# leabouffaut/DAS4Whales

Measured on AMD Instinct MI355X. Metric: channel-samples/sec through f-k filter + matched-filter, higher is better.
Workload: dtype f32 (matched filter: 2 x f16 split operands on the matrix cores, f32 accumulate); 1 GPU; 20000 channels x 120000 samples float32 per GPU, classic f-k fan mask (fk_filter_design defaults), stages fk+mf, HF+LF fin-call templates; api=public, parallelism=independent channel blocks x1

## Files before the change

das4whales_amd/csrc/mm_common.h:

```cpp
#pragma once
#include "fft_radix.h"

namespace d4w {

constexpr float kMmLoScale = 2048.f, kMmLoInv = 1.0f / 2048.f;

#ifdef D4W_EMU
typedef uint16_t mm_half;
struct alignas(16) mm_h8 { uint16_t v[8]; };
struct mm_f4 { float v[4]; };
__device__ __forceinline__ mm_half mm_to_half(float x) { return hipemu::f32_to_f16(x); }
__device__ __forceinline__ float mm_to_float(mm_half h) { return hipemu::f16_to_f32(h); }
__device__ __forceinline__ mm_f4 mm_zero() { return mm_f4{{0.f, 0.f, 0.f, 0.f}}; }
__device__ __forceinline__ mm_f4 mm_mfma(const mm_h8& a, const mm_h8& b, mm_f4 c) {
    hipemu::mfma_f32_16x16x32_f16(a.v, b.v, c.v);
    return c;
}
__device__ __forceinline__ float mm_get(const mm_f4& c, int r) { return c.v[r]; }
__device__ __forceinline__ void mm_set(mm_h8& a, int j, mm_half h) { a.v[j] = h; }
__device__ __forceinline__ int mm_uniform(int v) { return v; }
__device__ __forceinline__ void mm_sched_fence() {}
__device__ __forceinline__ void mm_store4(float* p, float a, float b, float c, float d) { p[0] = a; p[1] = b; p[2] = c; p[3] = d; }
__device__ __forceinline__ void mm_store1(float* p, float v) { *p = v; }
__device__ __forceinline__ float4 mm_load4_stream(const float4* p) { return *p; }
__device__ __forceinline__ void mm_put4(mm_half* p, const mm_half (&h)[4]) { p[0] = h[0]; p[1] = h[1]; p[2] = h[2]; p[3] = h[3]; }
__device__ __forceinline__ float mm_sqrt(float v) { return sqrtf(v); }
__device__ __forceinline__ void mm_wave_sync() { (void)__shfl_xor(0, 1); }
__device__ __forceinline__ float mm_clamp_half(float v) { return fminf(fmaxf(v, -65504.f), 65504.f); }
static inline int mm_num_cus() { return 2; }
#else
typedef _Float16 mm_half;
typedef _Float16 mm_h8 __attribute__((ext_vector_type(8)));
typedef _Float16 mm_h4 __attribute__((ext_vector_type(4)));
typedef float mm_f4 __attribute__((ext_vector_type(4)));
__device__ __forceinline__ mm_half mm_to_half(float x) { return (_Float16)x; }
__device__ __forceinline__ float mm_to_float(mm_half h) { return (float)h; }
__device__ __forceinline__ mm_f4 mm_zero() { mm_f4 z = {0.f, 0.f, 0.f, 0.f}; return z; }
__device__ __forceinline__ mm_f4 mm_mfma(mm_h8 a, mm_h8 b, mm_f4 c) { return __builtin_amdgcn_mfma_f32_16x16x32_f16(a, b, c, 0, 0, 0); }
__device__ __forceinline__ float mm_get(const mm_f4& c, int r) { return c[r]; }
__device__ __forceinline__ void mm_set(mm_h8& a, int j, mm_half h) { a[j] = h; }
__device__ __forceinline__ int mm_uniform(int v) { return __builtin_amdgcn_readfirstlane(v); }
__device__ __forceinline__ void mm_sched_fence() { __builtin_amdgcn_sched_barrier(0); }
__device__ __forceinline__ void mm_store4(float* p, float a, float b, float c, float d) {
    mm_f4 t = {a, b, c, d};
    __builtin_nontemporal_store(t, reinterpret_cast<mm_f4*>(p));
}
__device__ __forceinline__ void mm_store1(float* p, float v) { __builtin_nontemporal_store(v, p); }
__device__ __forceinline__ float4 mm_load4_stream(const float4* p) {
    const mm_f4 v = __builtin_nontemporal_load(reinterpret_cast<const mm_f4*>(p));
    return make_float4(v.x, v.y, v.z, v.w);
}
__device__ __forceinline__ void mm_put4(mm_half* p, const mm_half (&h)[4]) {
    mm_h4 v = {h[0], h[1], h[2], h[3]};
    *reinterpret_cast<mm_h4*>(p) = v;
}
__device__ __forceinline__ float mm_sqrt(float v) { return __builtin_amdgcn_sqrtf(v); }
__device__ __forceinline__ void mm_wave_sync() {
    __builtin_amdgcn_fence(__ATOMIC_RELEASE, "wavefront");
    __builtin_amdgcn_wave_barrier();
    __builtin_amdgcn_fence(__ATOMIC_ACQUIRE, "wavefront");
}
__device__ __forceinline__ float mm_clamp_half(float v) { return __builtin_amdgcn_fmed3f(v, -65504.f, 65504.f); }
static inline int mm_num_cus() {
    static int cached[64] = {0};
    int devid = 0, v = 0;
    if (hipGetDevice(&devid) != hipSuccess) return 256;
    if (devid >= 0 && devid < 64 && cached[devid] > 0) return cached[devid];
    if (hipDeviceGetAttribute(&v, hipDeviceAttributeMultiprocessorCount, devid) == hipSuccess && v > 0) {
        if (devid >= 0 && devid < 64) cached[devid] = v;
        return v;
    }
    return 256;
}
#endif

// ... 55 lines not shown
```

das4whales_amd/csrc/xcorr_mm.hip:

```cpp
#include <cstdlib>

#include "mm_common.h"

namespace d4w {

#ifndef D4W_MM_CH
#define D4W_MM_CH 4096
#endif
constexpr int kMmCH = D4W_MM_CH;
constexpr int kMmKS = 6;
constexpr int kMmKSLong = 8;
constexpr int kMmKSMax = 16;
constexpr int kMmSection = 32 * kMmKSMax - 16;
constexpr int kMmMaxSupport = 32 * kMmKSLong - 15;
constexpr int kMmMaxSections = 16;
constexpr int kMmThreads = 256;
template <int KSM>
struct MmGeom {
    static constexpr int Halo = 32 * KSM;
    static constexpr int Stage = kMmCH + Halo;
    static constexpr int Q = (Stage + 4 * kMmThreads - 1) / (4 * kMmThreads);
    static constexpr int LastQ = (Stage - (Q - 1) * 4 * kMmThreads) / 4;
    static constexpr int Arr = Stage + 8;
};
// ... 8 lines not shown
    float* y0;
    float* y1;
    int nx, ns, ld_next, n_next, ltaps, len0, len1;
    float* rowmax0;
    float* rowmax1;
    int clamp;
    int shift;
    int accumulate;
    float tail0, tail1;
};

__device__ __forceinline__ float mm_wave_scan(float v) {
#ifdef D4W_EMU
    const int lane = (int)(threadIdx.x & 63);
    for (int off = 1; off < 64; off <<= 1) {
        const float n = __shfl_up(v, (unsigned)off);
        if (lane >= off) v += n;
    }
    return v;
#else
    auto dpp = [](float x, auto ctrl, auto rmask) {
        return __int_as_float(__builtin_amdgcn_update_dpp(0, __float_as_int(x), decltype(ctrl)::value, decltype(rmask)::value, 0xf, false));
    };
    v += dpp(v, std::integral_constant<int, 0x111>{}, std::integral_constant<int, 0xf>{});
    v += dpp(v, std::integral_constant<int, 0x112>{}, std::integral_constant<int, 0xf>{});
    v += dpp(v, std::integral_constant<int, 0x114>{}, std::integral_constant<int, 0xf>{});
    v += dpp(v, std::integral_constant<int, 0x118>{}, std::integral_constant<int, 0xf>{});
    v += dpp(v, std::integral_constant<int, 0x142>{}, std::integral_constant<int, 0xa>{});
    v += dpp(v, std::integral_constant<int, 0x143>{}, std::integral_constant<int, 0xc>{});
    return v;
#endif
}

template <int KS0, int KS1, int WPS, bool TAIL = false, bool WMAX = false, bool WSPLIT = false>
__global__ __launch_bounds__(kMmThreads, WPS) void xcorr_mm_rows(MmArgs P) {
    static_assert(!(WSPLIT && KS1 > 0), "the wave-split kernel is the one-template code run by two wave pairs");
    constexpr int KSM = KS0 > KS1 ? KS0 : KS1;
    using GEO = MmGeom<KSM>;
    constexpr int kMmHalo = GEO::Halo, kMmStage = GEO::Stage, kMmQ = GEO::Q, kMmLastQ = GEO::LastQ, kMmArr = GEO::Arr;
    constexpr int kSeg = 4 * kMmQ;
    D4W_DYN_LDS(smem_raw);
    mm_half* lds = reinterpret_cast<mm_half*>(smem_raw);
    float* red = reinterpret_cast<float*>(lds + 4 * kMmArr);
    constexpr int kBlk = kMmCH / 4;
    float* pb = red + 8;
    float* wt = pb + 2 * kBlk;
    const int tid = (int)threadIdx.x;
    const int lane = tid & 63, wv = mm_uniform(tid >> 6);
    const int n16 = lane & 15, g = lane >> 4;
    const int ns = P.ns;
    const int tsel = WSPLIT ? (wv >> 1) : 0;

    const int nchunk = (ns + kMmCH - 1) / kMmCH;
    const long long total = (long long)P.nx * nchunk;
    const int nparts = min(8, (int)gridDim.x);
    const int xcd = (int)blockIdx.x % nparts, wq = (int)blockIdx.x / nparts, nq = ((int)gridDim.x - xcd + nparts - 1) / nparts;
    const long long lo_c = total * xcd / nparts, hi_c = total * (xcd + 1) / nparts;
    mm_h8 a0h[KS0], a0l[KS0];
    mm_h8 a1h[KS1 ? KS1 : 1], a1l[KS1 ? KS1 : 1];
    float osc0 = 1.f, osc1 = 1.f;
#ifdef D4W_MM_V_TAIL_DEALT
    constexpr bool kRows = false;
#else
    constexpr bool kRows = TAIL;
#endif
    auto next_chunk = [&](long long c) -> long long {
        if constexpr (kRows) {
            const long long r = c / nchunk;
            return (c - r * nchunk + 1 < nchunk) ? c + 1 : (r + (long long)gridDim.x) * nchunk;
        } else {
            return c + nq;
        }
    };
    const long long end_c = kRows ? total : hi_c;
    long long c_n = kRows ? (long long)blockIdx.x * nchunk : lo_c + wq;
    {
        float* tl = reinterpret_cast<float*>(smem_raw);
        constexpr int TLP = 16 + kMmHalo;
        for (int i = tid; i < 2 * TLP; i += kMmThreads) {
            const int t = i / TLP, u = i - t * TLP - 15;
            const int L = t ? P.len1 : P.len0;
            float tv = (u >= 0 && u < L && (t == 0 || KS1 > 0 || WSPLIT)) ? P.taps[(size_t)t * P.ltaps + u] : 0.f;
            if constexpr (TAIL) {
                if (u < L && (t == 0 || KS1 > 0 || WSPLIT)) tv += t ? P.tail1 : P.tail0;
            }
            tl[i] = tv;
        }
        __syncthreads();
        auto build = [&](const float* tp, int L, auto& ah, auto& al, auto ks, float& osc) {
            constexpr int KS = decltype(ks)::value;
            float m = 0.f;
            for (int i = lane; i < TLP; i += 64) m = fmaxf(m, fabsf(tp[i]));
            for (int o = 32; o > 0; o >>= 1) m = fmaxf(m, __shfl_xor(m, o));
            float up, down;
            mm_pow2_scale(m, up, down);
            osc = up;
            (void)L;
            static_for<KS>([&](auto kq) {
                constexpr int kk = decltype(kq)::value;
                static_for<8>([&](auto jq) {
                    constexpr int j = decltype(jq)::value;
                    const float v = tp[15 + 32 * kk + 8 * g + j - n16] * down;
                    mm_half hi, lo;
                    mm_split(v, hi, lo);
                    mm_set(ah[kk], j, hi);
                    mm_set(al[kk], j, lo);
                });
            });
        };
        build(tl + (WSPLIT ? tsel * TLP : 0), WSPLIT && tsel ? P.len1 : P.len0, a0h, a0l, std::integral_constant<int, KS0>{}, osc0);
        if constexpr (KS1 > 0) build(tl + TLP, P.len1, a1h, a1l, std::integral_constant<int, KS1>{}, osc1);
        __syncthreads();
    }

    float4 pre[kMmQ];
    Mean2 mu_n{0.f, 0.f};
    float g_n = 1.f;
    bool heavy_n = false;
    bool tail_n = false;
    int row_n = 0, c0_n = 0;

    auto issue = [&](long long c) {
        row_n = (int)(c / nchunk);
        c0_n = (int)(c - (long long)row_n * nchunk) * kMmCH;
        mu_n = mean2_load(P.mean, row_n);
        g_n = 1.f;
        const int s0 = c0_n + P.shift;
        tail_n = s0 + kMmStage > ns;
        if (P.maxabs) {
            const float a = P.maxabs[row_n];
            g_n = (a > 0.f) ? 1.0f / a : 0.f;
            heavy_n = fabsf(mu_n.hi) > 0.9921875f * a;
        }
        const float* xr = P.x + (size_t)row_n * ns;
        const bool al = (reinterpret_cast<uintptr_t>(xr + s0) & 15) == 0;
        if (al && s0 + kMmStage <= ns) {
            const float4* p = reinterpret_cast<const float4*>(xr + s0) + tid;
            static_for<kMmQ>([&](auto qq) {
                constexpr int q = decltype(qq)::value;
                if (q < kMmQ - 1 || tid < kMmLastQ) pre[q] = mm_load4_stream(p + q * kMmThreads);
            });
        } else {
            if (al && (ns & 3) == 0) {
                static_for<kMmQ>([&](auto qq) {
                    constexpr int q = decltype(qq)::value;
                    if (q < kMmQ - 1 || tid < kMmLastQ) {
                        const int i = s0 + 4 * (tid + q * kMmThreads);
                        const float4 v = *reinterpret_cast<const float4*>(xr + min(i, ns - 4));
                        pre[q] = (i < ns) ? v : make_float4(mu_n.hi, mu_n.hi, mu_n.hi, mu_n.hi);
                    }
                });
            } else {
                static_for<kMmQ>([&](auto qq) {
                    constexpr int q = decltype(qq)::value;
                    if (q < kMmQ - 1 || tid < kMmLastQ) {
                        const int i = s0 + 4 * (tid + q * kMmThreads);
                        const float a0 = xr[min(i, ns - 1)], a1 = xr[min(i + 1, ns - 1)], a2 = xr[min(i + 2, ns - 1)], a3 = xr[min(i + 3, ns - 1)];
                        pre[q] = make_float4(i < ns ? a0 : mu_n.hi, i + 1 < ns ? a1 : mu_n.hi, i + 2 < ns ? a2 : mu_n.hi, i + 3 < ns ? a3 : mu_n.hi);
                    }
                });
            }
            if (P.xnext && P.n_next > 0 && s0 + kMmStage > ns) {
                const float* xn = P.xnext + (size_t)row_n * P.ld_next;
                const int n_next = P.n_next;
                static_for<kMmQ>([&](auto qq) {
                    constexpr int q = decltype(qq)::value;
                    if (q < kMmQ - 1 || tid < kMmLastQ) {
                        const int d = s0 + 4 * (tid + q * kMmThreads) - ns;
                        const float b0 = xn[min(max(d, 0), n_next - 1)], b1 = xn[min(max(d + 1, 0), n_next - 1)];
                        const float b2 = xn[min(max(d + 2, 0), n_next - 1)], b3 = xn[min(max(d + 3, 0), n_next - 1)];
                        if (d >= 0 && d < n_next) pre[q].x = b0;
                        if (d + 1 >= 0 && d + 1 < n_next) pre[q].y = b1;
                        if (d + 2 >= 0 && d + 2 < n_next) pre[q].z = b2;
                        if (d + 3 >= 0 && d + 3 < n_next) pre[q].w = b3;
                    }
                });
            }
        }
    };

    if (c_n < end_c) issue(c_n);
    int buf = 0;
    constexpr bool want_max = WMAX;
    float pst_hi = 0.f, pst_lo = 0.f;
    for (long long c = c_n; c < end_c;) {
        const int row = row_n, c0 = c0_n;
        const Mean2 mu = mu_n;
        const bool tail = tail_n;
        const int n_valid = ns + ((P.xnext && P.n_next > 0) ? P.n_next : 0) - c0 - P.shift;
        float gsc = g_n, osx = 1.f;
        const float gout = g_n;
        const bool own_scale = !P.maxabs || heavy_n;
        mm_half* bh = lds + (size_t)buf * 2 * kMmArr;
        mm_half* bl = bh + kMmArr;
        const long long c_next = next_chunk(c);
        const int cin = c0 / kMmCH;
        if (TAIL && cin == 0) { pst_hi = 0.f; pst_lo = 0.f; }
        const float pst = pst_hi;
        if (own_scale) {
            float m = 0.f;
            static_for<kMmQ>([&](auto qq) {
                constexpr int q = decltype(qq)::value;
                if (q < kMmQ - 1 || tid < kMmLastQ) {
                    const float4 v = pre[q];
                    const int at = 4 * (tid + q * kMmThreads);
                    float d0 = demean(v.x, mu), d1 = demean(v.y, mu), d2 = demean(v.z, mu), d3 = demean(v.w, mu);
                    if (tail) {
                        if (at >= n_valid) d0 = 0.f;
                        if (at + 1 >= n_valid) d1 = 0.f;
                        if (at + 2 >= n_valid) d2 = 0.f;
                        if (at + 3 >= n_valid) d3 = 0.f;
                    }
                    m = fmaxf(fmaxf(m, fmaxf(fabsf(d0), fabsf(d1))), fmaxf(fabsf(d2), fabsf(d3)));
                }
            });
            for (int o = 32; o > 0; o >>= 1) m = fmaxf(m, __shfl_xor(m, o));
            if (lane == 0) red[wv + 4 * buf] = m;
            lds_barrier();
            m = fmaxf(fmaxf(red[4 * buf], red[4 * buf + 1]), fmaxf(red[4 * buf + 2], red[4 * buf + 3]));
            mm_pow2_scale(m, osx, gsc);
        }
        const float mlg = -mu.lo * gsc;
        static_for<kMmQ>([&](auto qq) {
            constexpr int q = decltype(qq)::value;
            float s[4] = {0.f, 0.f, 0.f, 0.f};
            const bool mine = q < kMmQ - 1 || tid < kMmLastQ;
            const int at = mm_pidx(4 * (tid + q * kMmThreads));
            if (mine) {
                const float4 v = pre[q];
#ifdef D4W_MM_V_FLOATMEAN
                s[0] = (v.x - mu.hi) * gsc; s[1] = (v.y - mu.hi) * gsc; s[2] = (v.z - mu.hi) * gsc; s[3] = (v.w - mu.hi) * gsc;
#else
                s[0] = fmaf(v.x - mu.hi, gsc, mlg); s[1] = fmaf(v.y - mu.hi, gsc, mlg); s[2] = fmaf(v.z - mu.hi, gsc, mlg); s[3] = fmaf(v.w - mu.hi, gsc, mlg);
#endif
                if (P.clamp && !own_scale) static_for<4>([&](auto ee) { constexpr int e = decltype(ee)::value; s[e] = mm_clamp_half(s[e]); });
                if (tail) {
                    const int a0 = 4 * (tid + q * kMmThreads);
                    static_for<4>([&](auto ee) { constexpr int e = decltype(ee)::value; if (a0 + e >= n_valid) s[e] = 0.f; });
                }
#ifdef D4W_MM_V_OLDSPLIT
                mm_half h[4], l[4];
                static_for<4>([&](auto ee) { constexpr int e = decltype(ee)::value; mm_split(s[e], h[e], l[e]); });
                mm_put4(bh + at, h);
                mm_put4(bl + at, l);
#else
                mm_split_put4(s, bh + at, bl + at);
#endif
            }
#ifdef D4W_MM_V_TAIL_NOSCAN
            if constexpr (false) {
#else
            if constexpr (TAIL && q < kMmCH / (4 * kMmThreads)) {
#endif
                const float t4 = (s[0] + s[1]) + (s[2] + s[3]);
                const float inc = mm_wave_scan(t4);
                pb[buf * kBlk + kMmThreads * q + tid] = inc - t4;
                if (lane == 63) wt[buf * 16 + 4 * q + wv] = inc;
            }
        });
        if (c_next < end_c) issue(c_next);
        lds_barrier();
        float* ya = ((WSPLIT && tsel) ? P.y1 : P.y0) + (size_t)row * ns;
        float* yb = KS1 ? P.y1 + (size_t)row * ns : nullptr;
        const bool valign = ((reinterpret_cast<uintptr_t>(ya + c0) & 15) == 0) && (!KS1 || (reinterpret_cast<uintptr_t>(yb + c0) & 15) == 0);
        const float oxs = (own_scale && P.maxabs) ? osx * gout : osx;
        const float o0 = osc0 * oxs, o1 = osc1 * oxs;
        float segoff = 0.f;
        constexpr int NTW = kMmCH / 256 / (WSPLIT ? 2 : 4), NST = NTW * KSM, PF = 2;
        auto tile_of = [&](int ti) { return WSPLIT ? (wv & 1) + 2 * ti : wv + 4 * ti; };
        auto frag = [&](const mm_half* arr, int T, int kk) -> mm_h8 {
            const int gr = 32 * T + 2 * n16 + g + 4 * kk;
            return *reinterpret_cast<const mm_h8*>(arr + mm_pidx(8 * gr));
        };
        mm_h8 fh[PF + 1], fl[PF + 1];
        static_for<PF>([&](auto ss) {
            constexpr int s_ = decltype(ss)::value;
            fh[s_] = frag(bh, tile_of(s_ / KSM), s_ % KSM);
            fl[s_] = frag(bl, tile_of(s_ / KSM), s_ % KSM);
        });
        mm_f4 c0h = mm_zero(), c0l = mm_zero(), c1h = mm_zero(), c1l = mm_zero();
        float vmax0 = -INFINITY, vmax1 = -INFINITY;
        float vsum = 0.f;
        static_for<NST>([&](auto ss) {
            constexpr int s_ = decltype(ss)::value, ti = s_ / KSM, kk = s_ % KSM;
            if constexpr (s_ + PF < NST) {
                fh[(s_ + PF) % (PF + 1)] = frag(bh, tile_of((s_ + PF) / KSM), (s_ + PF) % KSM);
                fl[(s_ + PF) % (PF + 1)] = frag(bl, tile_of((s_ + PF) / KSM), (s_ + PF) % KSM);
            }
            mm_sched_fence();
            const mm_h8 xh = fh[s_ % (PF + 1)], xl = fl[s_ % (PF + 1)];
            if constexpr (kk < KS0) {
                c0h = mm_mfma(a0h[kk], xh, c0h);
                c0l = mm_mfma(a0h[kk], xl, c0l);
            }
            if constexpr (kk < KS1) {
                c1h = mm_mfma(a1h[kk], xh, c1h);
                c1l = mm_mfma(a1h[kk], xl, c1l);
            }
            if constexpr (kk < KS0) c0l = mm_mfma(a0l[kk], xh, c0l);
            if constexpr (kk < KS1) c1l = mm_mfma(a1l[kk], xh, c1l);
            mm_sched_fence();
            if constexpr (kk == KSM - 1) {
                const int T = tile_of(ti);
                const int kl = 256 * T + 16 * n16 + 4 * g;
                const int k = c0 + kl;
                if constexpr (ti == 0) {
                if constexpr (TAIL) {
                    const float w = lane < 16 ? wt[buf * 16 + lane] : 0.f;
                    const float inc = mm_wave_scan(w);
                    segoff = inc - w;
        #ifdef D4W_EMU
                    const float own = __shfl(inc, 15);
        #else
                    const float own = __builtin_bit_cast(float, __builtin_amdgcn_readlane(__builtin_bit_cast(int, inc), 15));
        #endif
                    const double pd = ((double)pst_hi + (double)pst_lo) + (double)(own * oxs);
                    const float ph = (float)pd, pl2 = (float)(pd - (double)ph);
        #ifdef D4W_EMU
                    pst_hi = ph; pst_lo = pl2;
        #else
                    pst_hi = __builtin_bit_cast(float, __builtin_amdgcn_readfirstlane(__builtin_bit_cast(int, ph)));
                    pst_lo = __builtin_bit_cast(float, __builtin_amdgcn_readfirstlane(__builtin_bit_cast(int, pl2)));
        #endif
                }
                }
                float r0[4], r1[4];
                float a0 = 0.f, a1 = 0.f;
#ifdef D4W_MM_V_TAIL_NOSCAN
                if constexpr (false) {
#else
                if constexpr (TAIL) {
#endif
#ifdef D4W_EMU
                    const float so = __shfl(segoff, T);
#else
                    const float so = __builtin_bit_cast(float, __builtin_amdgcn_readlane(__builtin_bit_cast(int, segoff), T));
#endif
                    const float pbk = fmaf(so + pb[buf * kBlk + kMmThreads * (T >> 2) + 64 * (T & 3) + 4 * n16], oxs, pst);
                    a0 = ((WSPLIT && tsel) ? P.tail1 : P.tail0) * pbk;
                    a1 = P.tail1 * pbk;
                }
                static_for<4>([&](auto rr) {
                    constexpr int r = decltype(rr)::value;
                    r0[r] = fmaf(fmaf(mm_get(c0l, r), kMmLoInv, mm_get(c0h, r)), o0, a0);
                    if constexpr (KS1 > 0) r1[r] = fmaf(fmaf(mm_get(c1l, r), kMmLoInv, mm_get(c1h, r)), o1, a1);
                });
                c0h = mm_zero(); c0l = mm_zero(); c1h = mm_zero(); c1l = mm_zero();
                if (valign && k + 3 < ns) {
                    if (KS1 == 0 && P.accumulate) {
                        const float4 o = mm_load4_stream(reinterpret_cast<const float4*>(ya + k));
                        r0[0] += o.x; r0[1] += o.y; r0[2] += o.z; r0[3] += o.w;
                    }
                    mm_store4(ya + k, r0[0], r0[1], r0[2], r0[3]);
                    if constexpr (KS1 > 0) mm_store4(yb + k, r1[0], r1[1], r1[2], r1[3]);
                    if (want_max) {
                        vmax0 = fmaxf(vmax0, fmaxf(fmaxf(r0[0], r0[1]), fmaxf(r0[2], r0[3])));
#ifndef D4W_MM_V_NONAN
                        vsum += (r0[0] + r0[1]) + (r0[2] + r0[3]);
#endif
                        if constexpr (KS1 > 0) {
                            vmax1 = fmaxf(vmax1, fmaxf(fmaxf(r1[0], r1[1]), fmaxf(r1[2], r1[3])));
#ifndef D4W_MM_V_NONAN
                            vsum += (r1[0] + r1[1]) + (r1[2] + r1[3]);
#endif
                        }
                    }
                } else {
                    for (int r = 0; r < 4; ++r)
                        if (k + r < ns) {
                            const float v0 = (KS1 == 0 && P.accumulate) ? ya[k + r] + r0[r] : r0[r];
                            ya[k + r] = v0;
                            if constexpr (KS1 > 0) yb[k + r] = r1[r];
                            if (want_max) {
                                vmax0 = fmaxf(vmax0, v0);
                                vsum += v0;
                                if constexpr (KS1 > 0) { vmax1 = fmaxf(vmax1, r1[r]); vsum += r1[r]; }
                            }
                        }
                }
            }
        });
        if (want_max) {
            for (int o = 32; o > 0; o >>= 1) {
                vmax0 = fmaxf(vmax0, __shfl_xor(vmax0, o));
                if constexpr (KS1 > 0) vmax1 = fmaxf(vmax1, __shfl_xor(vmax1, o));
            }
            const bool bad = __any(vsum != vsum);
            if (lane == 0) {
                mm_atomic_fmax(((WSPLIT && tsel) ? P.rowmax1 : P.rowmax0) + row, bad ? __uint_as_float(0x7FC00000u) : vmax0);
                if constexpr (KS1 > 0) mm_atomic_fmax(P.rowmax1 + row, bad ? __uint_as_float(0x7FC00000u) : vmax1);
            }
        }
        buf ^= 1;
        c = c_next;
    }
}

}

using namespace d4w;

extern "C" {

int d4w_xcorr_mm_max_support(void) { return kMmSection * kMmMaxSections; }

#define D4W_MM_LAUNCH(KS0, KS1, WPS, TAIL, grid, lds, stream, Q)                                                              \
    do {                                                                                                                      \
        if ((Q).rowmax0) D4W_LAUNCH((xcorr_mm_rows<KS0, KS1, WPS, TAIL, true>), dim3(grid), dim3(kMmThreads), lds, stream, Q);  \
        else D4W_LAUNCH((xcorr_mm_rows<KS0, KS1, WPS, TAIL, false>), dim3(grid), dim3(kMmThreads), lds, stream, Q);             \
    } while (0)

static int mm_one_template(MmArgs P, const float* taps, int len, float* y, float* rowmax, int grid, void* stream) {
    auto lds_of = [](int arr) { return (size_t)4 * arr * sizeof(mm_half) + 8 * sizeof(float); };
    const int nsec = (len <= 32 * kMmKSMax - 15) ? 1 : ceil_div(len, kMmSection);
    const int per = (nsec == 1) ? len : 16 * ceil_div(ceil_div(len, nsec), 16);
    for (int j = 0; j < nsec; ++j) {
        const int first = j * per;
        MmArgs Q = P;
        Q.taps = taps + first;
        Q.len0 = Q.len1 = std::min(per, len - first);
        Q.y0 = y;
        Q.y1 = nullptr;
        Q.shift = first;
        Q.accumulate = j > 0;
        Q.rowmax0 = (j == nsec - 1) ? rowmax : nullptr;
        Q.rowmax1 = nullptr;
        const int ks = ceil_div(Q.len0 + 15, 32);
        if (ks <= kMmKS)
            D4W_MM_LAUNCH(kMmKS, 0, 3, false, grid, lds_of(MmGeom<kMmKS>::Arr), stream, Q);
        else if (ks <= kMmKSLong)
            D4W_MM_LAUNCH(kMmKSLong, 0, 2, false, grid, lds_of(MmGeom<kMmKSLong>::Arr), stream, Q);
        else if (ks <= 12)
            D4W_MM_LAUNCH(12, 0, 2, false, grid, lds_of(MmGeom<12>::Arr), stream, Q);
        else
            D4W_MM_LAUNCH(kMmKSMax, 0, 2, false, grid, lds_of(MmGeom<kMmKSMax>::Arr), stream, Q);
    }
    return D4W_OK;
}

int d4w_xcorr_mm_f32(const float* x, int nx, int ns, const float* xnext, int ld_next, int n_next, const double* mean,
                     const float* maxabs, const float* taps, int ntpl, int ltaps, int len0, int len1, float* y0, float* y1,
                     void* stream) {
    return d4w_xcorr_mm_rowmax_f32(x, nx, ns, xnext, ld_next, n_next, mean, maxabs, taps, ntpl, ltaps, len0, len1, y0, y1, nullptr,
// ... 9 lines not shown

int d4w_xcorr_mm_tail_max_support(void) { return 32 * kMmKSMax - 15; }

int d4w_xcorr_mm_tail_f32(const float* x, int nx, int ns, const float* xnext, int ld_next, int n_next, const double* mean,
                          const float* maxabs, const float* taps, int ntpl, int ltaps, int len0, int len1, double tail0, double tail1,
                          float* y0, float* y1, float* rowmax0, float* rowmax1, void* stream) {
    if (!x || !y0 || !taps || nx < 1 || ns < 1) return fail(D4W_EINVAL, "bad argument");
    if (ntpl == 2 && ((rowmax0 == nullptr) != (rowmax1 == nullptr))) return fail(D4W_EINVAL, "rowmax0 and rowmax1 go together");
    if (ntpl < 1 || ntpl > 2 || (ntpl == 2 && !y1)) return fail(D4W_EINVAL, "ntpl = %d (1 or 2 templates per call)", ntpl);
    if (xnext && (n_next < 0 || ld_next < n_next)) return fail(D4W_EINVAL, "a continuation needs 0 <= n_next <= ld_next");
    if (ntpl == 1) { len1 = len0; tail1 = 0.0; }
    if (len0 < 1 || len1 < 1 || len0 > ltaps || len1 > ltaps || std::max(len0, len1) > d4w_xcorr_mm_max_support())
        return fail(D4W_EINVAL, "template supports (%d, %d) must lie in 1..min(ltaps = %d, %d)", len0, len1, ltaps, d4w_xcorr_mm_max_support());
    const bool tails = tail0 != 0.0 || tail1 != 0.0;
    if (tails) {
        if (!mean || !maxabs) return fail(D4W_EINVAL, "the zero-padded template's tail needs the rows' statistics (mean, maxabs)");
        if (std::max(len0, len1) > d4w_xcorr_mm_tail_max_support())
            return fail(D4W_EINVAL, "with a tail the supports (%d, %d) must be <= %d", len0, len1, d4w_xcorr_mm_tail_max_support());
    }
    MmArgs P;
    P.x = x; P.xnext = xnext; P.mean = mean; P.maxabs = maxabs; P.taps = taps; P.y0 = y0; P.y1 = y1;
    P.nx = nx; P.ns = ns; P.ld_next = ld_next; P.n_next = xnext ? n_next : 0; P.ltaps = ltaps; P.len0 = len0; P.len1 = len1;
    P.shift = 0; P.accumulate = 0;
    static const int env_clamp = [] { const char* v = getenv("D4W_MM_CLAMP"); return v ? atoi(v) : 0; }();
    P.clamp = (xnext != nullptr && n_next > 0) || env_clamp;
    P.rowmax0 = rowmax0; P.rowmax1 = (ntpl == 2) ? rowmax1 : nullptr;
    P.tail0 = (float)tail0; P.tail1 = (float)tail1;
    if (rowmax0) {
        D4W_HIP(hipMemsetD32Async((hipDeviceptr_t)rowmax0, (int)0xFF800000u, (size_t)nx, (hipStream_t)stream));
        if (ntpl == 2) D4W_HIP(hipMemsetD32Async((hipDeviceptr_t)rowmax1, (int)0xFF800000u, (size_t)nx, (hipStream_t)stream));
    }
    const int nchunk = ceil_div(ns, kMmCH);
    const long long total = (long long)nx * nchunk;
    static const int env_wgs = [] { const char* v = getenv("D4W_MM_WGS"); const int n = v ? atoi(v) : 0; return n < 0 ? 0 : (n > 8 ? 8 : n); }();
    const int ks0 = ceil_div(len0 + 15, 32), ks1 = ceil_div(len1 + 15, 32);
    const bool fused = ntpl == 2 && std::max(ks0, ks1) <= kMmKS;
    const int per_cu = env_wgs ? env_wgs : ((ntpl == 1 && ks0 <= kMmKS) ? 3 : 2);
    const int ncu = mm_num_cus();
    const int grid = (int)std::min<long long>(total, (long long)ncu * per_cu);
    auto lds_of = [](int arr, bool tl) {
        return (size_t)4 * arr * sizeof(mm_half) + 8 * sizeof(float) + (tl ? ((size_t)2 * (kMmCH / 4) + 2 * 16) * sizeof(float) : 0);
    };
    static const int fused_form = [] { const char* v = getenv("D4W_MM_FUSED"); return v ? atoi(v) : 2; }();
    const int per_cu_ws = env_wgs ? env_wgs : 3;
#define D4W_MM_LAUNCH_WS(TAIL, grid, lds, Q)                                                                                            \
    do {                                                                                                                                \
        if ((Q).rowmax0) D4W_LAUNCH((xcorr_mm_rows<kMmKS, 0, 3, TAIL, true, true>), dim3(grid), dim3(kMmThreads), lds, stream, Q);       \
        else D4W_LAUNCH((xcorr_mm_rows<kMmKS, 0, 3, TAIL, false, true>), dim3(grid), dim3(kMmThreads), lds, stream, Q);                  \
    } while (0)
    if (tails) {
        const int grid_t = (int)std::min<long long>((long long)nx, (long long)ncu * per_cu);
        if (fused && fused_form != 2) {
            D4W_MM_LAUNCH_WS(true, (int)std::min<long long>((long long)nx, (long long)ncu * per_cu_ws), lds_of(MmGeom<kMmKS>::Arr, true), P);
            return D4W_OK;
        }
        if (fused) {
            const size_t lds = lds_of(MmGeom<kMmKS>::Arr, true);
            if (ks0 <= 5)
                D4W_MM_LAUNCH(5, kMmKS, 2, true, grid_t, lds, stream, P);
            else
                D4W_MM_LAUNCH(kMmKS, kMmKS, 2, true, grid_t, lds, stream, P);
            return D4W_OK;
        }
        for (int t = 0; t < ntpl; ++t) {
            MmArgs Q = P;
            Q.taps = taps + (size_t)t * ltaps;
            Q.len0 = Q.len1 = t ? len1 : len0;
            Q.tail0 = t ? (float)tail1 : (float)tail0;
            Q.tail1 = 0.f;
            Q.y0 = t ? y1 : y0;
            Q.y1 = nullptr;
            Q.rowmax0 = t ? rowmax1 : rowmax0;
            Q.rowmax1 = nullptr;
            const int ks = ceil_div(Q.len0 + 15, 32);
            if (ks <= kMmKS) {
                if (Q.rowmax0)
                    D4W_LAUNCH((xcorr_mm_rows<kMmKS, 0, 2, true, true>), dim3(grid_t), dim3(kMmThreads), lds_of(MmGeom<kMmKS>::Arr, true), stream, Q);
                else
                    D4W_LAUNCH((xcorr_mm_rows<kMmKS, 0, 3, true, false>), dim3(grid_t), dim3(kMmThreads), lds_of(MmGeom<kMmKS>::Arr, true), stream, Q);
            }
            else if (ks <= kMmKSLong)
                D4W_MM_LAUNCH(kMmKSLong, 0, 2, true, grid_t, lds_of(MmGeom<kMmKSLong>::Arr, true), stream, Q);
            else if (ks <= 12)
                D4W_MM_LAUNCH(12, 0, 2, true, grid_t, lds_of(MmGeom<12>::Arr, true), stream, Q);
            else
                D4W_MM_LAUNCH(kMmKSMax, 0, 2, true, grid_t, lds_of(MmGeom<kMmKSMax>::Arr, true), stream, Q);
        }
        return D4W_OK;
    }
    if (!fused) {
        int rc = mm_one_template(P, taps, len0, y0, rowmax0, grid, stream);
        if (rc == D4W_OK && ntpl == 2) rc = mm_one_template(P, taps + ltaps, len1, y1, rowmax1, grid, stream);
        return rc;
    }
    const size_t lds = lds_of(MmGeom<kMmKS>::Arr, false);
    if (fused_form != 2) {
        D4W_MM_LAUNCH_WS(false, (int)std::min<long long>(total, (long long)ncu * per_cu_ws), lds, P);
        return D4W_OK;
    }
    if (ks0 <= 5)
        D4W_MM_LAUNCH(5, kMmKS, 2, false, grid, lds, stream, P);
    else
        D4W_MM_LAUNCH(kMmKS, kMmKS, 2, false, grid, lds, stream, P);
    return D4W_OK;
}

}
```

Before: 114.3 billion channel-samples/s.

## Software-pipeline chunk conversion with MFMA matrix work in xcorr_mm_rows

Restructures the matched-filter kernel's chunk loop so the f16 hi/lo conversion of the next chunk is interleaved (sliced) into the MFMA matrix phase of the current chunk, using sched_group_barrier hints, rather than running convert and matrix back to back. Loading and conversion are split into locate/load/stats/convert lambdas, and chunk indices become 32-bit ints, with a host check rejecting inputs of more than 2^30 chunks. The pipelined variant is enabled by default via D4W_MM_PIPE, only for WPS==2 kernels whose KS is at most kMmKSLong. It risks higher register pressure and a more complex schedule, and falls back to the unsliced path for tail, clamp or own-scale chunks.

```diff
diff --git a/das4whales_amd/csrc/mm_common.h b/das4whales_amd/csrc/mm_common.h
--- a/das4whales_amd/csrc/mm_common.h
+++ b/das4whales_amd/csrc/mm_common.h
@@ -20,6 +20,7 @@
 __device__ __forceinline__ void mm_set(mm_h8& a, int j, mm_half h) { a.v[j] = h; }
 __device__ __forceinline__ int mm_uniform(int v) { return v; }
 __device__ __forceinline__ void mm_sched_fence() {}
+template <int MASK, int N> __device__ __forceinline__ void mm_sched_group() {}
 __device__ __forceinline__ void mm_store4(float* p, float a, float b, float c, float d) { p[0] = a; p[1] = b; p[2] = c; p[3] = d; }
 __device__ __forceinline__ void mm_store1(float* p, float v) { *p = v; }
 __device__ __forceinline__ float4 mm_load4_stream(const float4* p) { return *p; }
@@ -41,6 +42,7 @@
 __device__ __forceinline__ void mm_set(mm_h8& a, int j, mm_half h) { a[j] = h; }
 __device__ __forceinline__ int mm_uniform(int v) { return __builtin_amdgcn_readfirstlane(v); }
 __device__ __forceinline__ void mm_sched_fence() { __builtin_amdgcn_sched_barrier(0); }
+template <int MASK, int N> __device__ __forceinline__ void mm_sched_group() { __builtin_amdgcn_sched_group_barrier(MASK, N, 0); }
 __device__ __forceinline__ void mm_store4(float* p, float a, float b, float c, float d) {
     mm_f4 t = {a, b, c, d};
     __builtin_nontemporal_store(t, reinterpret_cast<mm_f4*>(p));
diff --git a/das4whales_amd/csrc/xcorr_mm.hip b/das4whales_amd/csrc/xcorr_mm.hip
--- a/das4whales_amd/csrc/xcorr_mm.hip
+++ b/das4whales_amd/csrc/xcorr_mm.hip
@@ -64,7 +64,7 @@
 #endif
 }
 
-template <int KS0, int KS1, int WPS, bool TAIL = false, bool WMAX = false, bool WSPLIT = false>
+template <int KS0, int KS1, int WPS, bool TAIL = false, bool WMAX = false, bool WSPLIT = false, bool PIPE = true>
 __global__ __launch_bounds__(kMmThreads, WPS) void xcorr_mm_rows(MmArgs P) {
     static_assert(!(WSPLIT && KS1 > 0), "the wave-split kernel is the one-template code run by two wave pairs");
     constexpr int KSM = KS0 > KS1 ? KS0 : KS1;
@@ -84,10 +84,10 @@
     const int tsel = WSPLIT ? (wv >> 1) : 0;
 
     const int nchunk = (ns + kMmCH - 1) / kMmCH;
-    const long long total = (long long)P.nx * nchunk;
+    const int total = P.nx * nchunk;
     const int nparts = min(8, (int)gridDim.x);
     const int xcd = (int)blockIdx.x % nparts, wq = (int)blockIdx.x / nparts, nq = ((int)gridDim.x - xcd + nparts - 1) / nparts;
-    const long long lo_c = total * xcd / nparts, hi_c = total * (xcd + 1) / nparts;
+    const int lo_c = (int)((long long)total * xcd / nparts), hi_c = (int)((long long)total * (xcd + 1) / nparts);
     mm_h8 a0h[KS0], a0l[KS0];
     mm_h8 a1h[KS1 ? KS1 : 1], a1l[KS1 ? KS1 : 1];
     float osc0 = 1.f, osc1 = 1.f;
@@ -96,16 +96,16 @@
 #else
     constexpr bool kRows = TAIL;
 #endif
-    auto next_chunk = [&](long long c) -> long long {
+    auto next_chunk = [&](int c) -> int {
         if constexpr (kRows) {
-            const long long r = c / nchunk;
-            return (c - r * nchunk + 1 < nchunk) ? c + 1 : (r + (long long)gridDim.x) * nchunk;
+            const int r = c / nchunk;
+            return (c - r * nchunk + 1 < nchunk) ? c + 1 : (r + (int)gridDim.x) * nchunk;
         } else {
             return c + nq;
         }
     };
-    const long long end_c = kRows ? total : hi_c;
-    long long c_n = kRows ? (long long)blockIdx.x * nchunk : lo_c + wq;
+    const int end_c = kRows ? total : hi_c;
+    const int c_n = kRows ? (int)blockIdx.x * nchunk : lo_c + wq;
     {
         float* tl = reinterpret_cast<float*>(smem_raw);
         constexpr int TLP = 16 + kMmHalo;
@@ -146,159 +146,194 @@
     }
 
     float4 pre[kMmQ];
-    Mean2 mu_n{0.f, 0.f};
-    float g_n = 1.f;
-    bool heavy_n = false;
-    bool tail_n = false;
     int row_n = 0, c0_n = 0;
-
-    auto issue = [&](long long c) {
-        row_n = (int)(c / nchunk);
-        c0_n = (int)(c - (long long)row_n * nchunk) * kMmCH;
-        mu_n = mean2_load(P.mean, row_n);
-        g_n = 1.f;
+    bool fast_n = false;
+    auto locate = [&](int c) {
+        row_n = c / nchunk;
+        c0_n = (c - row_n * nchunk) * kMmCH;
         const int s0 = c0_n + P.shift;
-        tail_n = s0 + kMmStage > ns;
-        if (P.maxabs) {
-            const float a = P.maxabs[row_n];
-            g_n = (a > 0.f) ? 1.0f / a : 0.f;
-            heavy_n = fabsf(mu_n.hi) > 0.9921875f * a;
-        }
+        fast_n = ((reinterpret_cast<uintptr_t>(P.x + (size_t)row_n * ns + s0) & 15) == 0) && s0 + kMmStage <= ns;
+    };
+    auto load_fast = [&](auto qq) {
+        constexpr int q = decltype(qq)::value;
+        if (q < kMmQ - 1 || tid < kMmLastQ)
+            pre[q] = mm_load4_stream(reinterpret_cast<const float4*>(P.x + (size_t)row_n * ns + c0_n + P.shift) + tid + q * kMmThreads);
+    };
+    auto load_all = [&]() {
+        if (fast_n) {
+            static_for<kMmQ>(load_fast);
+            return;
+        }
+        const int s0 = c0_n + P.shift;
         const float* xr = P.x + (size_t)row_n * ns;
+        const float fill = mean2_load(P.mean, row_n).hi;
         const bool al = (reinterpret_cast<uintptr_t>(xr + s0) & 15) == 0;
-        if (al && s0 + kMmStage <= ns) {
-            const float4* p = reinterpret_cast<const float4*>(xr + s0) + tid;
+        if (al && (ns & 3) == 0) {
             static_for<kMmQ>([&](auto qq) {
                 constexpr int q = decltype(qq)::value;
-                if (q < kMmQ - 1 || tid < kMmLastQ) pre[q] = mm_load4_stream(p + q * kMmThreads);
+                if (q < kMmQ - 1 || tid < kMmLastQ) {
+                    const int i = s0 + 4 * (tid + q * kMmThreads);
+                    const float4 v = *reinterpret_cast<const float4*>(xr + min(i, ns - 4));
+                    pre[q] = (i < ns) ? v : make_float4(fill, fill, fill, fill);
+                }
             });
         } else {
-            if (al && (ns & 3) == 0) {
-                static_for<kMmQ>([&](auto qq) {
-                    constexpr int q = decltype(qq)::value;
-                    if (q < kMmQ - 1 || tid < kMmLastQ) {
-                        const int i = s0 + 4 * (tid + q * kMmThreads);
-                        const float4 v = *reinterpret_cast<const float4*>(xr + min(i, ns - 4));
-                        pre[q] = (i < ns) ? v : make_float4(mu_n.hi, mu_n.hi, mu_n.hi, mu_n.hi);
-                    }
-                });
-            } else {
-                static_for<kMmQ>([&](auto qq) {
-                    constexpr int q = decltype(qq)::value;
-                    if (q < kMmQ - 1 || tid < kMmLastQ) {
-                        const int i = s0 + 4 * (tid + q * kMmThreads);
-                        const float a0 = xr[min(i, ns - 1)], a1 = xr[min(i + 1, ns - 1)], a2 = xr[min(i + 2, ns - 1)], a3 = xr[min(i + 3, ns - 1)];
-                        pre[q] = make_float4(i < ns ? a0 : mu_n.hi, i + 1 < ns ? a1 : mu_n.hi, i + 2 < ns ? a2 : mu_n.hi, i + 3 < ns ? a3 : mu_n.hi);
-                    }
-                });
-            }
-            if (P.xnext && P.n_next > 0 && s0 + kMmStage > ns) {
-                const float* xn = P.xnext + (size_t)row_n * P.ld_next;
-                const int n_next = P.n_next;
-                static_for<kMmQ>([&](auto qq) {
-                    constexpr int q = decltype(qq)::value;
-                    if (q < kMmQ - 1 || tid < kMmLastQ) {
-                        const int d = s0 + 4 * (tid + q * kMmThreads) - ns;
-                        const float b0 = xn[min(max(d, 0), n_next - 1)], b1 = xn[min(max(d + 1, 0), n_next - 1)];
-                        const float b2 = xn[min(max(d + 2, 0), n_next - 1)], b3 = xn[min(max(d + 3, 0), n_next - 1)];
-                        if (d >= 0 && d < n_next) pre[q].x = b0;
-                        if (d + 1 >= 0 && d + 1 < n_next) pre[q].y = b1;
-                        if (d + 2 >= 0 && d + 2 < n_next) pre[q].z = b2;
-                        if (d + 3 >= 0 && d + 3 < n_next) pre[q].w = b3;
-                    }
-                });
-            }
-        }
-    };
-
-    if (c_n < end_c) issue(c_n);
-    int buf = 0;
-    constexpr bool want_max = WMAX;
-    float pst_hi = 0.f, pst_lo = 0.f;
-    for (long long c = c_n; c < end_c;) {
-        const int row = row_n, c0 = c0_n;
-        const Mean2 mu = mu_n;
-        const bool tail = tail_n;
-        const int n_valid = ns + ((P.xnext && P.n_next > 0) ? P.n_next : 0) - c0 - P.shift;
-        float gsc = g_n, osx = 1.f;
-        const float gout = g_n;
-        const bool own_scale = !P.maxabs || heavy_n;
-        mm_half* bh = lds + (size_t)buf * 2 * kMmArr;
-        mm_half* bl = bh + kMmArr;
-        const long long c_next = next_chunk(c);
-        const int cin = c0 / kMmCH;
-        if (TAIL && cin == 0) { pst_hi = 0.f; pst_lo = 0.f; }
-        const float pst = pst_hi;
-        if (own_scale) {
+            static_for<kMmQ>([&](auto qq) {
+                constexpr int q = decltype(qq)::value;
+                if (q < kMmQ - 1 || tid < kMmLastQ) {
+                    const int i = s0 + 4 * (tid + q * kMmThreads);
+                    const float a0 = xr[min(i, ns - 1)], a1 = xr[min(i + 1, ns - 1)], a2 = xr[min(i + 2, ns - 1)], a3 = xr[min(i + 3, ns - 1)];
+                    pre[q] = make_float4(i < ns ? a0 : fill, i + 1 < ns ? a1 : fill, i + 2 < ns ? a2 : fill, i + 3 < ns ? a3 : fill);
+                }
+            });
+        }
+        if (P.xnext && P.n_next > 0 && s0 + kMmStage > ns) {
+            const float* xn = P.xnext + (size_t)row_n * P.ld_next;
+            const int n_next = P.n_next;
+            static_for<kMmQ>([&](auto qq) {
+                constexpr int q = decltype(qq)::value;
+                if (q < kMmQ - 1 || tid < kMmLastQ) {
+                    const int d = s0 + 4 * (tid + q * kMmThreads) - ns;
+                    const float b0 = xn[min(max(d, 0), n_next - 1)], b1 = xn[min(max(d + 1, 0), n_next - 1)];
+                    const float b2 = xn[min(max(d + 2, 0), n_next - 1)], b3 = xn[min(max(d + 3, 0), n_next - 1)];
+                    if (d >= 0 && d < n_next) pre[q].x = b0;
+                    if (d + 1 >= 0 && d + 1 < n_next) pre[q].y = b1;
+                    if (d + 2 >= 0 && d + 2 < n_next) pre[q].z = b2;
+                    if (d + 3 >= 0 && d + 3 < n_next) pre[q].w = b3;
+                }
+            });
+        }
+    };
+
+    Mean2 mu_k{0.f, 0.f};
+    float g_k = 1.f, gsc_k = 1.f, mlg_k = 0.f;
+    bool own_k = false;
+    bool tail_k = false, clamp_k = false;
+    int nvalid_k = 0, buf_k = 0;
+    auto stats_k = [&](int row, int c0) {
+        mu_k = mean2_load(P.mean, row);
+        g_k = 1.f;
+        own_k = !P.maxabs;
+        if (P.maxabs) {
+            const float a = P.maxabs[row];
+            g_k = (a > 0.f) ? 1.0f / a : 0.f;
+            own_k = fabsf(mu_k.hi) > 0.9921875f * a;
+        }
+        tail_k = c0 + P.shift + kMmStage > ns;
+        nvalid_k = ns + ((P.xnext && P.n_next > 0) ? P.n_next : 0) - c0 - P.shift;
+        clamp_k = P.clamp && !own_k;
+        gsc_k = g_k;
+        mlg_k = -mu_k.lo * gsc_k;
+    };
+    float cs[4];
+    auto conv_part = [&](auto qq, auto pp, auto edge) {
+        constexpr int q = decltype(qq)::value, part = decltype(pp)::value;
+        constexpr bool EDGE = decltype(edge)::value;
+        const bool mine = q < kMmQ - 1 || tid < kMmLastQ;
+        mm_half* bh = lds + (size_t)buf_k * 2 * kMmArr;
+        const int a0 = 4 * (tid + q * kMmThreads);
+        if constexpr (part == 0) {
+            cs[0] = cs[1] = cs[2] = cs[3] = 0.f;
+            if (mine) {
+                const float4 v = pre[q];
+#ifdef D4W_MM_V_FLOATMEAN
+                cs[0] = (v.x - mu_k.hi) * gsc_k; cs[1] = (v.y - mu_k.hi) * gsc_k; cs[2] = (v.z - mu_k.hi) * gsc_k; cs[3] = (v.w - mu_k.hi) * gsc_k;
+#else
+                cs[0] = fmaf(v.x - mu_k.hi, gsc_k, mlg_k); cs[1] = fmaf(v.y - mu_k.hi, gsc_k, mlg_k);
+                cs[2] = fmaf(v.z - mu_k.hi, gsc_k, mlg_k); cs[3] = fmaf(v.w - mu_k.hi, gsc_k, mlg_k);
+#endif
+                if constexpr (EDGE) {
+                    if (clamp_k) static_for<4>([&](auto ee) { constexpr int e = decltype(ee)::value; cs[e] = mm_clamp_half(cs[e]); });
+                    if (tail_k)
+                        static_for<4>([&](auto ee) { constexpr int e = decltype(ee)::value; if (a0 + e >= nvalid_k) cs[e] = 0.f; });
+                }
+            }
+        } else if constexpr (part == 1) {
+            if (mine) {
+#ifdef D4W_MM_V_OLDSPLIT
+                mm_half h[4], l[4];
+                static_for<4>([&](auto ee) { constexpr int e = decltype(ee)::value; mm_split(cs[e], h[e], l[e]); });
+                mm_put4(bh + mm_pidx(a0), h);
+                mm_put4(bh + kMmArr + mm_pidx(a0), l);
+#else
+                mm_split_put4(cs, bh + mm_pidx(a0), bh + kMmArr + mm_pidx(a0));
+#endif
+            }
+        } else {
+#ifdef D4W_MM_V_TAIL_NOSCAN
+            if constexpr (false) {
+#else
+            if constexpr (TAIL && q < kMmCH / (4 * kMmThreads)) {
+#endif
+                const float t4 = (cs[0] + cs[1]) + (cs[2] + cs[3]);
+                const float inc = mm_wave_scan(t4);
+                pb[buf_k * kBlk + kMmThreads * q + tid] = inc - t4;
+                if (lane == 63) wt[buf_k * 16 + 4 * q + wv] = inc;
+            }
+        }
+    };
+    auto convert_all = [&]() -> float {
+        float osx = 1.f;
+        if (own_k) {
             float m = 0.f;
             static_for<kMmQ>([&](auto qq) {
                 constexpr int q = decltype(qq)::value;
                 if (q < kMmQ - 1 || tid < kMmLastQ) {
                     const float4 v = pre[q];
                     const int at = 4 * (tid + q * kMmThreads);
-                    float d0 = demean(v.x, mu), d1 = demean(v.y, mu), d2 = demean(v.z, mu), d3 = demean(v.w, mu);
-                    if (tail) {
-                        if (at >= n_valid) d0 = 0.f;
-                        if (at + 1 >= n_valid) d1 = 0.f;
-                        if (at + 2 >= n_valid) d2 = 0.f;
-                        if (at + 3 >= n_valid) d3 = 0.f;
+                    float d0 = demean(v.x, mu_k), d1 = demean(v.y, mu_k), d2 = demean(v.z, mu_k), d3 = demean(v.w, mu_k);
+                    if (tail_k) {
+                        if (at >= nvalid_k) d0 = 0.f;
+                        if (at + 1 >= nvalid_k) d1 = 0.f;
+                        if (at + 2 >= nvalid_k) d2 = 0.f;
+                        if (at + 3 >= nvalid_k) d3 = 0.f;
                     }
                     m = fmaxf(fmaxf(m, fmaxf(fabsf(d0), fabsf(d1))), fmaxf(fabsf(d2), fabsf(d3)));
                 }
             });
             for (int o = 32; o > 0; o >>= 1) m = fmaxf(m, __shfl_xor(m, o));
-            if (lane == 0) red[wv + 4 * buf] = m;
+            if (lane == 0) red[wv + 4 * buf_k] = m;
             lds_barrier();
-            m = fmaxf(fmaxf(red[4 * buf], red[4 * buf + 1]), fmaxf(red[4 * buf + 2], red[4 * buf + 3]));
-            mm_pow2_scale(m, osx, gsc);
-        }
-        const float mlg = -mu.lo * gsc;
-        static_for<kMmQ>([&](auto qq) {
-            constexpr int q = decltype(qq)::value;
-            float s[4] = {0.f, 0.f, 0.f, 0.f};
-            const bool mine = q < kMmQ - 1 || tid < kMmLastQ;
-            const int at = mm_pidx(4 * (tid + q * kMmThreads));
-            if (mine) {
-                const float4 v = pre[q];
-#ifdef D4W_MM_V_FLOATMEAN
-                s[0] = (v.x - mu.hi) * gsc; s[1] = (v.y - mu.hi) * gsc; s[2] = (v.z - mu.hi) * gsc; s[3] = (v.w - mu.hi) * gsc;
-#else
-                s[0] = fmaf(v.x - mu.hi, gsc, mlg); s[1] = fmaf(v.y - mu.hi, gsc, mlg); s[2] = fmaf(v.z - mu.hi, gsc, mlg); s[3] = fmaf(v.w - mu.hi, gsc, mlg);
-#endif
-                if (P.clamp && !own_scale) static_for<4>([&](auto ee) { constexpr int e = decltype(ee)::value; s[e] = mm_clamp_half(s[e]); });
-                if (tail) {
-                    const int a0 = 4 * (tid + q * kMmThreads);
-                    static_for<4>([&](auto ee) { constexpr int e = decltype(ee)::value; if (a0 + e >= n_valid) s[e] = 0.f; });
-                }
-#ifdef D4W_MM_V_OLDSPLIT
-                mm_half h[4], l[4];
-                static_for<4>([&](auto ee) { constexpr int e = decltype(ee)::value; mm_split(s[e], h[e], l[e]); });
-                mm_put4(bh + at, h);
-                mm_put4(bl + at, l);
-#else
-                mm_split_put4(s, bh + at, bl + at);
-#endif
-            }
-#ifdef D4W_MM_V_TAIL_NOSCAN
-            if constexpr (false) {
-#else
-            if constexpr (TAIL && q < kMmCH / (4 * kMmThreads)) {
-#endif
-                const float t4 = (s[0] + s[1]) + (s[2] + s[3]);
-                const float inc = mm_wave_scan(t4);
-                pb[buf * kBlk + kMmThreads * q + tid] = inc - t4;
-                if (lane == 63) wt[buf * 16 + 4 * q + wv] = inc;
+            m = fmaxf(fmaxf(red[4 * buf_k], red[4 * buf_k + 1]), fmaxf(red[4 * buf_k + 2], red[4 * buf_k + 3]));
+            mm_pow2_scale(m, osx, gsc_k);
+            mlg_k = -mu_k.lo * gsc_k;
+        }
+        auto all = [&](auto edge) {
+            static_for<kMmQ>([&](auto qq) {
+                static_for<3>([&](auto pp) { conv_part(qq, pp, edge); });
+            });
+        };
+        if (tail_k || clamp_k) all(std::true_type{});
+        else all(std::false_type{});
+        return (own_k && P.maxabs) ? osx * g_k : osx;
+    };
+    constexpr int NPART = TAIL ? 4 : 3, NPC = kMmQ * NPART;
+    auto conv_slice = [&](auto ss, auto nstq) {
+        constexpr int s_ = decltype(ss)::value, nst = decltype(nstq)::value;
+        static_for<NPC>([&](auto pq) {
+            constexpr int p = decltype(pq)::value, q = p / NPART, part = p % NPART;
+            if constexpr (p * nst / NPC == s_) {
+                if constexpr (part == NPART - 1) load_fast(std::integral_constant<int, q>{});
+                else conv_part(std::integral_constant<int, q>{}, std::integral_constant<int, part>{}, std::false_type{});
             }
         });
-        if (c_next < end_c) issue(c_next);
-        lds_barrier();
+    };
+    auto no_slice = [](auto, auto) {};
+
+    float pst_hi = 0.f, pst_lo = 0.f;
+    auto matrix = [&](int row, int c0, float oxs, int buf, auto slice) {
+        mm_half* bh = lds + (size_t)buf * 2 * kMmArr;
+        mm_half* bl = bh + kMmArr;
+        const int cin = c0 / kMmCH;
+        if (TAIL && cin == 0) { pst_hi = 0.f; pst_lo = 0.f; }
+        const float pst = pst_hi;
         float* ya = ((WSPLIT && tsel) ? P.y1 : P.y0) + (size_t)row * ns;
         float* yb = KS1 ? P.y1 + (size_t)row * ns : nullptr;
         const bool valign = ((reinterpret_cast<uintptr_t>(ya + c0) & 15) == 0) && (!KS1 || (reinterpret_cast<uintptr_t>(yb + c0) & 15) == 0);
-        const float oxs = (own_scale && P.maxabs) ? osx * gout : osx;
         const float o0 = osc0 * oxs, o1 = osc1 * oxs;
         float segoff = 0.f;
         constexpr int NTW = kMmCH / 256 / (WSPLIT ? 2 : 4), NST = NTW * KSM, PF = 2;
+        static_assert(NPC <= NST, "at most one part of the conversion per k-step");
         auto tile_of = [&](int ti) { return WSPLIT ? (wv & 1) + 2 * ti : wv + 4 * ti; };
         auto frag = [&](const mm_half* arr, int T, int kk) -> mm_h8 {
             const int gr = 32 * T + 2 * n16 + g + 4 * kk;
@@ -331,30 +366,35 @@
             }
             if constexpr (kk < KS0) c0l = mm_mfma(a0l[kk], xh, c0l);
             if constexpr (kk < KS1) c1l = mm_mfma(a1l[kk], xh, c1l);
+            slice(ss, std::integral_constant<int, NST>{});
+            static_for<(kk < KS0 ? 3 : 0) + (kk < KS1 ? 3 : 0)>([&](auto) {
+                mm_sched_group<0x8, 1>();
+                mm_sched_group<0x2, 2>();
+            });
             mm_sched_fence();
             if constexpr (kk == KSM - 1) {
                 const int T = tile_of(ti);
                 const int kl = 256 * T + 16 * n16 + 4 * g;
                 const int k = c0 + kl;
                 if constexpr (ti == 0) {
-                if constexpr (TAIL) {
-                    const float w = lane < 16 ? wt[buf * 16 + lane] : 0.f;
-                    const float inc = mm_wave_scan(w);
-                    segoff = inc - w;
-        #ifdef D4W_EMU
-                    const float own = __shfl(inc, 15);
-        #else
-                    const float own = __builtin_bit_cast(float, __builtin_amdgcn_readlane(__builtin_bit_cast(int, inc), 15));
-        #endif
-                    const double pd = ((double)pst_hi + (double)pst_lo) + (double)(own * oxs);
-                    const float ph = (float)pd, pl2 = (float)(pd - (double)ph);
-        #ifdef D4W_EMU
-                    pst_hi = ph; pst_lo = pl2;
-        #else
-                    pst_hi = __builtin_bit_cast(float, __builtin_amdgcn_readfirstlane(__builtin_bit_cast(int, ph)));
-                    pst_lo = __builtin_bit_cast(float, __builtin_amdgcn_readfirstlane(__builtin_bit_cast(int, pl2)));
-        #endif
-                }
+                    if constexpr (TAIL) {
+                        const float w = lane < 16 ? wt[buf * 16 + lane] : 0.f;
+                        const float inc = mm_wave_scan(w);
+                        segoff = inc - w;
+#ifdef D4W_EMU
+                        const float own = __shfl(inc, 15);
+#else
+                        const float own = __builtin_bit_cast(float, __builtin_amdgcn_readlane(__builtin_bit_cast(int, inc), 15));
+#endif
+                        const double pd = ((double)pst_hi + (double)pst_lo) + (double)(own * oxs);
+                        const float ph = (float)pd, pl2 = (float)(pd - (double)ph);
+#ifdef D4W_EMU
+                        pst_hi = ph; pst_lo = pl2;
+#else
+                        pst_hi = __builtin_bit_cast(float, __builtin_amdgcn_readfirstlane(__builtin_bit_cast(int, ph)));
+                        pst_lo = __builtin_bit_cast(float, __builtin_amdgcn_readfirstlane(__builtin_bit_cast(int, pl2)));
+#endif
+                    }
                 }
                 float r0[4], r1[4];
                 float a0 = 0.f, a1 = 0.f;
@@ -385,7 +425,7 @@
                     }
                     mm_store4(ya + k, r0[0], r0[1], r0[2], r0[3]);
                     if constexpr (KS1 > 0) mm_store4(yb + k, r1[0], r1[1], r1[2], r1[3]);
-                    if (want_max) {
+                    if (WMAX) {
                         vmax0 = fmaxf(vmax0, fmaxf(fmaxf(r0[0], r0[1]), fmaxf(r0[2], r0[3])));
 #ifndef D4W_MM_V_NONAN
                         vsum += (r0[0] + r0[1]) + (r0[2] + r0[3]);
@@ -403,7 +443,7 @@
                             const float v0 = (KS1 == 0 && P.accumulate) ? ya[k + r] + r0[r] : r0[r];
                             ya[k + r] = v0;
                             if constexpr (KS1 > 0) yb[k + r] = r1[r];
-                            if (want_max) {
+                            if (WMAX) {
                                 vmax0 = fmaxf(vmax0, v0);
                                 vsum += v0;
                                 if constexpr (KS1 > 0) { vmax1 = fmaxf(vmax1, r1[r]); vsum += r1[r]; }
@@ -412,7 +452,7 @@
                 }
             }
         });
-        if (want_max) {
+        if (WMAX) {
             for (int o = 32; o > 0; o >>= 1) {
                 vmax0 = fmaxf(vmax0, __shfl_xor(vmax0, o));
                 if constexpr (KS1 > 0) vmax1 = fmaxf(vmax1, __shfl_xor(vmax1, o));
@@ -423,8 +463,60 @@
                 if constexpr (KS1 > 0) mm_atomic_fmax(P.rowmax1 + row, bad ? __uint_as_float(0x7FC00000u) : vmax1);
             }
         }
-        buf ^= 1;
-        c = c_next;
+    };
+
+    if constexpr (!PIPE) {
+        if (c_n < end_c) { locate(c_n); load_all(); }
+        int buf = 0;
+        for (int c = c_n; c < end_c;) {
+            const int row = row_n, c0 = c0_n;
+            stats_k(row, c0);
+            buf_k = buf;
+            const float oxs = convert_all();
+            const int c_next = next_chunk(c);
+            if (c_next < end_c) { locate(c_next); load_all(); }
+            lds_barrier();
+            matrix(row, c0, oxs, buf, no_slice);
+            buf ^= 1;
+            c = c_next;
+        }
+    } else {
+        int c = c_n;
+        int row_m = 0, c0_m = 0, buf = 0;
+        float oxs_m = 1.f;
+        if (c < end_c) {
+            locate(c);
+            load_all();
+            row_m = row_n; c0_m = c0_n;
+            stats_k(row_m, c0_m);
+            buf_k = 0;
+            oxs_m = convert_all();
+            const int c1 = next_chunk(c);
+            if (c1 < end_c) { locate(c1); load_all(); }
+            lds_barrier();
+        }
+        while (c < end_c) {
+            const int c_next = next_chunk(c);
+            const bool have_k = c_next < end_c;
+            const int row_k = row_n, c0_k = c0_n;
+            if (have_k) { stats_k(row_k, c0_k); buf_k = buf ^ 1; }
+            const int c_nn = have_k ? next_chunk(c_next) : end_c;
+            if (c_nn < end_c) locate(c_nn);
+            float oxs_k = 1.f;
+            if (have_k && !own_k && !tail_k && !clamp_k && c_nn < end_c && fast_n) {
+                matrix(row_m, c0_m, oxs_m, buf, conv_slice);
+            } else {
+                matrix(row_m, c0_m, oxs_m, buf, no_slice);
+                if (have_k) {
+                    oxs_k = convert_all();
+                    if (c_nn < end_c) load_all();
+                }
+            }
+            lds_barrier();
+            row_m = row_k; c0_m = c0_k; oxs_m = oxs_k;
+            buf ^= 1;
+            c = c_next;
+        }
     }
 }
 
@@ -432,15 +524,38 @@
 
 using namespace d4w;
 
+static bool mm_pipe() {
+    static const bool on = [] { const char* v = getenv("D4W_MM_PIPE"); return !v || atoi(v) != 0; }();
+    return on;
+}
+template <int KS0, int KS1, int WPS>
+constexpr bool mm_pipe_fits() { return WPS == 2 && (KS0 > KS1 ? KS0 : KS1) <= kMmKSLong; }
+template <int KS0, int KS1, int WPS, bool TAIL, bool WMAX, bool WSPLIT>
+static int mm_launch(int grid, size_t lds, void* stream, const MmArgs& Q) {
+    if constexpr (mm_pipe_fits<KS0, KS1, WPS>()) {
+        if (mm_pipe()) {
+            D4W_LAUNCH((xcorr_mm_rows<KS0, KS1, WPS, TAIL, WMAX, WSPLIT, true>), dim3(grid), dim3(kMmThreads), lds, stream, Q);
+            return D4W_OK;
+        }
+    }
+    D4W_LAUNCH((xcorr_mm_rows<KS0, KS1, WPS, TAIL, WMAX, WSPLIT, false>), dim3(grid), dim3(kMmThreads), lds, stream, Q);
+    return D4W_OK;
+}
+#define D4W_MM_LAUNCH_P(KS0, KS1, WPS, TAIL, WMAX, WSPLIT, grid, lds, stream, Q)                        \
+    do {                                                                                              \
+        const int rc_ = mm_launch<KS0, KS1, WPS, TAIL, WMAX, WSPLIT>((grid), (lds), (stream), (Q));   \
+        if (rc_ != D4W_OK) return rc_;                                                                \
+    } while (0)
+#define D4W_MM_LAUNCH(KS0, KS1, WPS, TAIL, grid, lds, stream, Q)                       \
+    do {                                                                               \
+        if ((Q).rowmax0) D4W_MM_LAUNCH_P(KS0, KS1, WPS, TAIL, true, false, grid, lds, stream, Q); \
+        else D4W_MM_LAUNCH_P(KS0, KS1, WPS, TAIL, false, false, grid, lds, stream, Q);            \
+    } while (0)
+
+
 extern "C" {
 
 int d4w_xcorr_mm_max_support(void) { return kMmSection * kMmMaxSections; }
-
-#define D4W_MM_LAUNCH(KS0, KS1, WPS, TAIL, grid, lds, stream, Q)                                                              \
-    do {                                                                                                                      \
-        if ((Q).rowmax0) D4W_LAUNCH((xcorr_mm_rows<KS0, KS1, WPS, TAIL, true>), dim3(grid), dim3(kMmThreads), lds, stream, Q);  \
-        else D4W_LAUNCH((xcorr_mm_rows<KS0, KS1, WPS, TAIL, false>), dim3(grid), dim3(kMmThreads), lds, stream, Q);             \
-    } while (0)
 
 static int mm_one_template(MmArgs P, const float* taps, int len, float* y, float* rowmax, int grid, void* stream) {
     auto lds_of = [](int arr) { return (size_t)4 * arr * sizeof(mm_half) + 8 * sizeof(float); };
@@ -516,6 +631,7 @@
     }
     const int nchunk = ceil_div(ns, kMmCH);
     const long long total = (long long)nx * nchunk;
+    if (total >= (1LL << 30)) return fail(D4W_EINVAL, "%d x %d samples: more than 2^30 chunks of %d", nx, ns, kMmCH);
     static const int env_wgs = [] { const char* v = getenv("D4W_MM_WGS"); const int n = v ? atoi(v) : 0; return n < 0 ? 0 : (n > 8 ? 8 : n); }();
     const int ks0 = ceil_div(len0 + 15, 32), ks1 = ceil_div(len1 + 15, 32);
     const bool fused = ntpl == 2 && std::max(ks0, ks1) <= kMmKS;
@@ -529,8 +645,8 @@
     const int per_cu_ws = env_wgs ? env_wgs : 3;
 #define D4W_MM_LAUNCH_WS(TAIL, grid, lds, Q)                                                                                            \
     do {                                                                                                                                \
-        if ((Q).rowmax0) D4W_LAUNCH((xcorr_mm_rows<kMmKS, 0, 3, TAIL, true, true>), dim3(grid), dim3(kMmThreads), lds, stream, Q);       \
-        else D4W_LAUNCH((xcorr_mm_rows<kMmKS, 0, 3, TAIL, false, true>), dim3(grid), dim3(kMmThreads), lds, stream, Q);                  \
+        if ((Q).rowmax0) D4W_MM_LAUNCH_P(kMmKS, 0, 3, TAIL, true, true, grid, lds, stream, Q);                                         \
+        else D4W_MM_LAUNCH_P(kMmKS, 0, 3, TAIL, false, true, grid, lds, stream, Q);                                                    \
     } while (0)
     if (tails) {
         const int grid_t = (int)std::min<long long>((long long)nx, (long long)ncu * per_cu);
@@ -559,9 +675,9 @@
             const int ks = ceil_div(Q.len0 + 15, 32);
             if (ks <= kMmKS) {
                 if (Q.rowmax0)
-                    D4W_LAUNCH((xcorr_mm_rows<kMmKS, 0, 2, true, true>), dim3(grid_t), dim3(kMmThreads), lds_of(MmGeom<kMmKS>::Arr, true), stream, Q);
+                    D4W_MM_LAUNCH_P(kMmKS, 0, 2, true, true, false, grid_t, lds_of(MmGeom<kMmKS>::Arr, true), stream, Q);
                 else
-                    D4W_LAUNCH((xcorr_mm_rows<kMmKS, 0, 3, true, false>), dim3(grid_t), dim3(kMmThreads), lds_of(MmGeom<kMmKS>::Arr, true), stream, Q);
+                    D4W_MM_LAUNCH_P(kMmKS, 0, 3, true, false, false, grid_t, lds_of(MmGeom<kMmKS>::Arr, true), stream, Q);
             }
             else if (ks <= kMmKSLong)
                 D4W_MM_LAUNCH(kMmKSLong, 0, 2, true, grid_t, lds_of(MmGeom<kMmKSLong>::Arr, true), stream, Q);
```

Result: no change. 114.3 billion channel-samples/s, median of 6 (+0.0%).
